# gardnerzhou/CHAP

Hardware: AMD Instinct MI355X
Metric: training volumes/sec (2D 256^2 bs24) (higher is better)
Workload: dtype bf16; 1 GPU; ACDC 2D DualDecoder bs=24 (12 lab + 12 unlab) 256x256, 1 perturb step(s), N_v=U; global_batch=24, parallelism=dp1, hip_graph=True, losses_finite=True

## Files before the change

chap_amd/csrc/conv_api.hip:

```cpp
#include <cstdlib>
#include <atomic>
#include "common.h"
#include "launch.h"

int chap_conv_launch_kpar_bf16(const chap_conv_params* p, int KC, int cpar, hipStream_t s);
int chap_conv_launch_wp_bf16(const chap_conv_params* p, int KC, hipStream_t s);
#define DECL_GEOM(dt, g) int chap_conv_launch_##dt##_g##g(const chap_conv_params* p, int KC, int NT, int MR, hipStream_t s);
DECL_GEOM(bf16, 1) DECL_GEOM(bf16, 2) DECL_GEOM(bf16, 3) DECL_GEOM(bf16, 4) DECL_GEOM(bf16, 5)
DECL_GEOM(f32, 1) DECL_GEOM(f32, 2) DECL_GEOM(f32, 3) DECL_GEOM(f32, 4) DECL_GEOM(f32, 5)
typedef int (*conv_launch_fn)(const chap_conv_params*, int, int, int, hipStream_t);

struct conv_blocking { int KC, GPT, NP, STEPS, nchunks, ntiles; };

static conv_blocking blocking_for(int Ck, int taps, int Cout_logical, int dtype) {
    conv_blocking b;
    b.KC = (Ck >= 32 && Ck % 32 == 0) ? 32 : 16;
    (void)dtype;
    {
        static int kc16_maxc = -1, kc16_maxc2 = -1;
        if (kc16_maxc < 0) { const char* e = getenv("CHAP_CONV_KC16_MAXC"); kc16_maxc = (e && atoi(e) > 0) ? atoi(e) : 1 << 20; }
        if (kc16_maxc2 < 0) { const char* e = getenv("CHAP_CONV_KC16_MAXC2D"); kc16_maxc2 = (e && atoi(e) > 0) ? atoi(e) : 0; }
        if (taps == 27 && Ck >= 32 && Ck <= kc16_maxc) b.KC = 16;
        if (taps == 9 && Ck >= 32 && Ck <= kc16_maxc2) b.KC = 16;
    }
// ... 54 lines not shown
                   "chap_conv_fwd: input dims (%d,%d,%d) do not match grid (%d,%d,%d) stride %d", p->ID, p->IH, p->IW, p->D, p->H, p->W, p->stride);
    if (p->dims == 3 && (p->src[0].keep || (p->nsrc > 1 && p->src[1].keep))) { chap_set_error("chap_conv_fwd: element keep masks are built for 2D only (3D: channel multipliers)"); return CHAP_EUNSUPPORTED; }
    if (p->out_mode == 1) CHAP_CHECK_ARG(p->out_Cn > 0 && p->out_Cn % 16 == 0 && p->Cout % p->out_Cn == 0, "chap_conv_fwd: depth-to-space needs Cn%%16==0");
    if (!p->out_planar) CHAP_CHECK_ARG(p->out_ld % 4 == 0 && p->out_coff % 4 == 0, "chap_conv_fwd: out_ld/out_coff must be multiples of 4");
    if (p->out2) CHAP_CHECK_ARG(p->out_mode == 0 && !p->out_planar && !p->out_f32 && (p->Cout & 3) == 0 && p->out2_from > 0 && p->out2_from % 16 == 0 && p->out2_from < p->Cout &&
                                p->ksize == 3 && p->stride == 1, "chap_conv_fwd: out2 needs a channel-last k3 s1 output, out2_from %% 16 == 0 inside (0, Cout)");
    const int Ck = p->combine == 0 ? p->src[0].C + (p->nsrc > 1 ? p->src[1].C : 0) : p->src[0].C;
    const int taps = p->ksize * p->ksize * (p->dims == 3 ? p->ksize : 1);
    conv_blocking b = blocking_for(Ck, taps, p->Cout, p->dtype);
    CHAP_CHECK_ARG(Ck % b.KC == 0, "chap_conv_fwd: K channels %d not a multiple of %d", Ck, b.KC);
    const bool d3 = p->dims == 3;
    int geom;
    if (p->ksize == 3 && p->stride == 1) geom = d3 ? 2 : 1;
    else if (p->ksize == 1 && p->stride == 1) geom = 3;
    else if (p->ksize == 2 && p->stride == 2) geom = d3 ? 5 : 4;
    else { chap_set_error("chap_conv_fwd: unsupported (ksize=%d, stride=%d)", p->ksize, p->stride); return CHAP_EUNSUPPORTED; }
    if (p->combine == 1 && p->nsrc == 2 && geom != 2 && geom != 1) { chap_set_error("chap_conv_fwd: add-combine is built for k3 s1 only"); return CHAP_EUNSUPPORTED; }
    int NT = b.ntiles >= 4 ? 4 : (b.ntiles >= 2 ? 2 : 1);
    int MR = (geom == 2 || geom == 5) ? 1 : 2;
    const bool bf = p->dtype == CHAP_BF16;
    if (geom == 2 && bf) {
        const long bricks = (long)p->N * cdiv(p->D, 4) * cdiv(p->H, 4) * cdiv(p->W, 16);
        if (bricks >= 64) {
            MR = 4;
            if (NT > 2) NT = 2;
            while (NT > 1 && bricks * cdiv(b.ntiles, NT) < 128) NT >>= 1;
        } else if (b.KC == 32 && NT > 2) {
            NT = 2;
        }
    }
    if (geom == 1 || geom == 3) {
        auto blocks = [&](int mr, int nt) { return (long)p->N * p->D * cdiv(p->H, 4 * mr) * cdiv(p->W, 16) * cdiv(b.ntiles, nt); };
        if (geom == 1 && bf && b.KC == 32 && b.ntiles >= 4) {
            MR = 2; NT = 2;
        } else if (geom == 1 && b.KC == 16 && blocks(4, NT) >= 512) MR = 4;
        else if (blocks(2, NT) >= 384) MR = 2;
        else {
            MR = 1;
            while (NT > 1 && blocks(1, NT) < 384) NT >>= 1;
        }
    }
    {
        const char* ent = getenv("CHAP_CONV_NT"); const char* emr = getenv("CHAP_CONV_MR"); const char* emc = getenv("CHAP_CONV_MINC");
        const int minc = emc ? atoi(emc) : 64;
        if ((geom == 1 || geom == 2) && Ck >= minc) {
            if (ent && atoi(ent) > 0 && atoi(ent) <= b.ntiles) NT = atoi(ent);
            if (emr && atoi(emr) > 0) MR = atoi(emr);
        }
    }
    if (p->dtype == CHAP_BF16 && geom == 3 && p->out_planar && p->Cout <= 8 && p->nsrc == 1 && Ck == 16 && p->src[0].C == 16 && !p->stats && p->out_mode == 0) {
        const long total = (long)p->N * p->D * p->H * p->W;
        return chap_launch<chap_conv_params, conv_head1x1_kernel<bf16_t>, 256>(dim3(chap_blocks(total, 4096)), dim3(256), 0, (hipStream_t)stream, *p, "chap_conv_fwd(head)");
    }
    if (p->dtype == CHAP_BF16 && geom == 1 && p->out_mode == 0 && !p->out_planar && !p->out_f32 && (p->Cout & 15) == 0 && p->Cout <= 64 && p->combine == 0 &&
        Ck == b.KC && (p->nsrc == 1 || (b.KC == 32 && p->src[0].C == 16 && p->src[1].C == 16))) {
        const char* ew = getenv("CHAP_CONV_WP");
        const long wp_min = ew ? atol(ew) : 1;
        const long t4 = (long)p->N * cdiv(p->H, 4) * cdiv(p->W, 16);
        if (wp_min > 0 && t4 >= wp_min) return chap_conv_launch_wp_bf16(p, b.KC, (hipStream_t)stream);
    }
    if (p->dtype == CHAP_BF16 && (geom == 1 || geom == 2) && p->out_mode == 0 && !p->out_planar && (p->Cout & 3) == 0 && !p->out2 &&
        (p->nsrc == 1 || (p->combine == 0 && p->src[0].C % b.KC == 0)) && !(d3 && (p->src[0].keep || (p->nsrc > 1 && p->src[1].keep)))) {
        const char* ek = getenv("CHAP_CONV_KPAR");
        const int mode = ek ? atoi(ek) : 2;
        const int cpar = b.nchunks % 4 == 0 ? 4 : (b.nchunks % 2 == 0 ? 2 : 0);
        const long kblocks = (long)p->N * p->D * cdiv(p->H, d3 ? 4 : 8) * cdiv(p->W, 16) * cdiv(b.ntiles, 2);
        const char* ekm = getenv("CHAP_CONV_KPAR_MAX");
        const long kmax = ekm ? atol(ekm) : 800;
        if (cpar && Ck >= 64 && (mode == 1 || (mode == 2 && d3 && kblocks <= kmax))) return chap_conv_launch_kpar_bf16(p, b.KC, cpar, (hipStream_t)stream);
    }
    static const conv_launch_fn table[2][5] = {
        {chap_conv_launch_f32_g1, chap_conv_launch_f32_g2, chap_conv_launch_f32_g3, chap_conv_launch_f32_g4, chap_conv_launch_f32_g5},
        {chap_conv_launch_bf16_g1, chap_conv_launch_bf16_g2, chap_conv_launch_bf16_g3, chap_conv_launch_bf16_g4, chap_conv_launch_bf16_g5}};
    if (p->dtype != CHAP_BF16 && p->dtype != CHAP_F32) { chap_set_error("chap_conv_fwd: dtype=%d", p->dtype); return CHAP_EINVAL; }
    return table[p->dtype == CHAP_BF16][geom - 1](p, b.KC, NT, MR, (hipStream_t)stream);
}

struct pack_geom { int Ck, Ck_real, Cn_logical, ctaps; };
static int pack_geometry(const chap_pack_params* p, pack_geom* g) {
    switch (p->kind) {
        case CHAP_PACK_CONV_FWD:     g->Ck = p->Cin;  g->Cn_logical = p->Cout;           g->ctaps = p->taps; break;
        case CHAP_PACK_CONV_DGRAD:   g->Ck = p->Cout; g->Cn_logical = p->Cin;            g->ctaps = p->taps; break;
        case CHAP_PACK_DECONV_FWD:   g->Ck = p->Cin;  g->Cn_logical = p->taps * p->Cout; g->ctaps = 1;       break;
        case CHAP_PACK_DECONV_DGRAD: g->Ck = p->Cout; g->Cn_logical = p->Cin;            g->ctaps = p->taps; break;
        case CHAP_PACK_DOWN_DGRAD:   g->Ck = p->Cout; g->Cn_logical = p->taps * p->Cin;  g->ctaps = 1;       break;
        default: chap_set_error("chap_pack: kind=%d", p->kind); return CHAP_EINVAL;
    }
    g->Ck_real = g->Ck;
    g->Ck = (g->Ck + 15) / 16 * 16;
    return CHAP_OK;
}

template <typename T>
__device__ __forceinline__ void pack_body(const float* __restrict__ w, T* __restrict__ out, int kind, int Cin, int Cout, int taps,
                                          int KC, int GPT, int NP, int STEPS, int nchunks, int ntiles, int Cn_logical, int Ck_real,
                                          long first, long stride) {
    const long total = (long)nchunks * STEPS * ntiles * 64;
    const int PPS = STEPS * 4;
    for (long q = first; q < total; q += stride) {
        const int pp = (int)(q % PPS);
        long r = q / PPS;
        const int n16 = (int)(r & 15); r >>= 4;
        const int nt = (int)(r % ntiles);
        const int chunk = (int)(r / ntiles);
        const int step = pp >> 2, g = pp & 3;
        const long i = ((long)(chunk * STEPS + step) * ntiles + nt) * 64 + g * 16 + n16;
        const int nl = nt * 16 + n16;
        float v[8];
// ... 90 lines not shown
```

chap_amd/csrc/conv_wp.h:

```cpp
#pragma once
#include "conv_kernel.h"
#include "wgrad_wp.h"

constexpr int CWP_AFFC = 64;

template <int KC, int NT>
__host__ __device__ constexpr size_t conv_wp_lds_bytes() {
    typedef conv_geom<3, 1, false, 1, false> G;
    constexpr int GPT = KC / 8, NP = G::NTAPS * GPT, STEPS = (NP + 3) / 4;
    return (size_t)STEPS * NT * 512 * sizeof(bf16_t)
           + 4 * ((size_t)G::HP * pix_stride<bf16_t, KC>() + HALO_DUMMY) * sizeof(bf16_t)
           + 4 * 2 * 16 * NT * sizeof(float) + 2 * CWP_AFFC * sizeof(float) + 2 * 16 * NT * sizeof(float);
}

template <int KC, int NT, bool LANESEL>
__device__ __forceinline__ void conv_wp_kernel(const chap_conv_params& P) {
    typedef bf16_t T;
    typedef conv_geom<3, 1, false, 1, false> G;
    typedef typename frag<T>::type F;
    constexpr int GPT = KC / 8, PS = pix_stride<T, KC>();
    constexpr int NP = G::NTAPS * GPT, STEPS = (NP + 3) / 4;
    constexpr int UNITS = (G::HP * GPT + 63) / 64;
    constexpr int ROWS = G::TH;
    constexpr size_t HB = (size_t)G::HP * PS + HALO_DUMMY;
    static_assert((HB * sizeof(T)) % 16 == 0, "the float4 reads of bc need a 16-byte aligned tail");
    extern __shared__ __attribute__((aligned(16))) char smem[];
    T* wlds = (T*)smem;
    const int lane = threadIdx.x & 63, wave = threadIdx.x >> 6;
    T* halo = wlds + (size_t)STEPS * NT * 512 + wave * HB;
    float* bstat = (float*)(wlds + (size_t)STEPS * NT * 512 + 4 * HB);
    float* aff = bstat + 4 * 2 * 16 * NT;
    float* bc = aff + 2 * CWP_AFFC;
    const int px = lane & 15, g = lane >> 4;
    const int tiles_x = (P.W + G::TW - 1) / G::TW, tiles_y = (P.H + G::TH - 1) / G::TH;
    const long ntiles = (long)P.N * tiles_y * tiles_x;
    const int ntiles_total = (P.Cout + 15) >> 4;
    const int nt0 = blockIdx.y * NT;
    const bool one = P.nsrc == 1;
    const bool plain = P.src[0].scale == nullptr && !P.src[0].act && P.src[0].keep == nullptr && P.src[0].chan_mul == nullptr &&
                       (one || (P.src[1].scale == nullptr && !P.src[1].act && P.src[1].keep == nullptr && P.src[1].chan_mul == nullptr));
    const src_scalars s0 = make_scalars(P.src[0]);
    const src_scalars s1 = make_scalars(one ? P.src[0] : P.src[1]);
    const bool do_stats = P.stats != nullptr;

    const int nb = gridDim.x;
    const int NG = nb < 8 ? nb : 8;
    const int xcd = blockIdx.x % NG;
    const int sj = ((int)blockIdx.x / NG) * 4 + wave;
    const int bpx = ((nb + NG - 1 - xcd) / NG) * 4;
    const long per = (ntiles + NG - 1) / NG;
    const long t_lo = per * xcd, t_hi = t_lo + per < ntiles ? t_lo + per : ntiles;
    const long my_tiles = (bpx > 0 && t_lo + sj < t_hi) ? (t_hi - t_lo - sj + bpx - 1) / bpx : 0;
    const long last_tile = t_lo + sj + (my_tiles > 0 ? my_tiles - 1 : 0) * bpx;
    auto tile_of = [&](long k) __attribute__((always_inline)) { const long t = t_lo + sj + k * bpx; return t < last_tile ? t : last_tile; };

    unit_desc<UNITS> U;
    make_units_wave<G, GPT, PS, UNITS>(U, P.IH, P.IW, lane);
    halo_regs<T, UNITS, false, true> R;
    int n = 0, y0 = 0, x0 = 0, nn = 0, ny0 = 0, nx0 = 0;
    auto issue = [&](long tile) __attribute__((always_inline)) {
        int z0_;
        tile_coords<G::TH, G::TW, 1>(tile, tiles_x, tiles_y, 1, nn, z0_, ny0, nx0);
        halo_issue_impl<T, G, false, 1, KC, false, UNITS, LANESEL, false>(R, U, s0, s1, 1, P.IH, P.IW, nn, 0, ny0, nx0, 0);
    };
    if (my_tiles > 0) issue(tile_of(0));
    float asc[2], ash[2];
    {
        const int s_ = threadIdx.x >> 5, c = threadIdx.x & 31;
        const chap_src_t& S = P.src[(s_ < P.nsrc && s_ < 2) ? s_ : 0];
        const int cc = c < S.C ? c : 0;
        asc[0] = S.scale ? S.scale[cc] : 1.f; ash[0] = S.scale ? S.shift[cc] : 0.f;
        asc[1] = 0.f; ash[1] = 0.f;
    }
    const long wstep = (long)ntiles_total * 64 * 8;
    constexpr int WPT = (STEPS * NT * 64 + 255) / 256;
    F wreg[WPT];
#pragma unroll
    for (int k = 0; k < WPT; ++k) {
        const unsigned i = min((unsigned)(threadIdx.x + 256 * k), (unsigned)(STEPS * NT * 64 - 1));
        const unsigned ln = i & 63u, r = i >> 6, t = r % (unsigned)NT, step = r / (unsigned)NT;
        const unsigned tt = nt0 + (int)t < ntiles_total ? t : 0u;
        wreg[k] = frag<T>::load((const T*)P.wpacked + (long)step * wstep + ((long)(nt0 + tt) * 64 + ln) * 8);
    }
    float ssum[NT][4], ssq[NT][4];
#pragma unroll
    for (int t = 0; t < NT; ++t)
#pragma unroll
        for (int j = 0; j < 4; ++j) { ssum[t][j] = 0.f; ssq[t][j] = 0.f; }
    float bcv = 0.f;
    if (threadIdx.x < 2 * 16 * NT) {
        const int which = threadIdx.x / (16 * NT), nl = nt0 * 16 + (int)threadIdx.x % (16 * NT);
        const float* srcp = which == 0 ? P.bias : (do_stats ? P.stats_shift : nullptr);
        if (srcp != nullptr && nl < P.Cout) bcv = srcp[nl];
    }
    if (threadIdx.x < 64) {
        const int s_ = threadIdx.x >> 5, c = threadIdx.x & 31;
        aff[s_ * CWP_AFFC + c] = asc[0]; aff[s_ * CWP_AFFC + CWP_AFFC / 2 + c] = ash[0];
    }
    if (threadIdx.x < 2 * 16 * NT) bc[threadIdx.x] = bcv;
#pragma unroll
    for (int k = 0; k < WPT; ++k) {
        const unsigned i = threadIdx.x + 256 * k;
        if (i < (unsigned)(STEPS * NT * 64)) {
            const unsigned t = (i >> 6) % (unsigned)NT;
            frag<T>::store(wlds + (size_t)i * 8, (nt0 + (int)t < ntiles_total) ? wreg[k] : frag<T>::zero());
        }
    }
    int xoff[STEPS];
#pragma unroll
    for (int step = 0; step < STEPS; ++step) {
        const int p = step * 4 + g;
        const int tap = p / GPT, cgl = p % GPT;
        const int dx = tap % 3, dy = tap / 3;
        xoff[step] = p < NP ? ((dy * G::HW) + px + dx) * PS + cgl * 8 : -1;
    }
    int ooff[NT];
#pragma unroll
    for (int t = 0; t < NT; ++t) {
        const int nl = (nt0 + t) * 16 + 4 * g;
        ooff[t] = px * P.out_ld + P.out_coff + ((P.out2 && nl >= P.out2_from) ? nl - P.out2_from : nl);
    }
    const int orow = P.W * P.out_ld;
    __syncthreads();
    if (my_tiles > 0) {
        halo_commit_impl<T, KC, false, UNITS, LANESEL, true, false, CWP_AFFC>(R, U, halo, s0, s1, aff, plain, nn, 0);
        for (long k = 0;; ++k) {
            n = nn; y0 = ny0; x0 = nx0;
            issue(tile_of(k + 1));
            f32x4 acc[ROWS][NT];
#pragma unroll
            for (int m = 0; m < ROWS; ++m)
#pragma unroll
                for (int t = 0; t < NT; ++t) acc[m][t] = (f32x4){0.f, 0.f, 0.f, 0.f};
#pragma unroll
            for (int step = 0; step < STEPS; ++step) {
                F wf[NT], xf[ROWS];
#pragma unroll
                for (int t = 0; t < NT; ++t) wf[t] = frag<T>::load(wlds + ((size_t)(step * NT + t) * 64 + lane) * 8);
                const int xo = xoff[step];
#pragma unroll
                for (int m = 0; m < ROWS; ++m) {
                    if (step * 4 + 3 < NP) xf[m] = frag<T>::load(halo + xo + m * (G::HW * PS));
                    else xf[m] = xo >= 0 ? frag<T>::load(halo + xo + m * (G::HW * PS)) : frag<T>::zero();
                }
#pragma unroll
                for (int m = 0; m < ROWS; ++m)
#pragma unroll
                    for (int t = 0; t < NT; ++t) mma8(acc[m][t], wf[t], xf[m]);
            }
            {
                const bool xok = x0 + px < P.W;
                const long o0 = (((long)n * P.H + y0) * P.W + x0) * P.out_ld;
                char* ob = (char*)P.out + o0 * (long)sizeof(T);
                char* ob2 = P.out2 ? (char*)P.out2 + o0 * (long)sizeof(T) : ob;
#pragma unroll
                for (int t = 0; t < NT; ++t) {
                    const bool cok = (nt0 + t) * 16 + 4 * g < P.Cout;
                    char* obt = (P.out2 && (nt0 + t) * 16 >= P.out2_from) ? ob2 : ob;
                    const float4 b4 = *(const float4*)(bc + t * 16 + 4 * g), c4 = *(const float4*)(bc + 16 * NT + t * 16 + 4 * g);
                    const float bj[4] = {b4.x, b4.y, b4.z, b4.w}, cj[4] = {c4.x, c4.y, c4.z, c4.w};
#pragma unroll
                    for (int m = 0; m < ROWS; ++m) {
                        const bool valid = xok && cok && (y0 + m < P.H);
                        float v[4];
#pragma unroll
                        for (int j = 0; j < 4; ++j) v[j] = acc[m][t][j] + bj[j];
                        if (do_stats) {
#pragma unroll
                            for (int j = 0; j < 4; ++j) { const float d = valid ? v[j] - cj[j] : 0.f; ssum[t][j] += d; ssq[t][j] += d * d; }
                        }
                        if (valid) st4((T*)(obt + (unsigned)(m * orow + ooff[t]) * (unsigned)sizeof(T)), v);
                    }
                }
            }
            if (k + 1 >= my_tiles) break;
            halo_commit_impl<T, KC, false, UNITS, LANESEL, true, false, CWP_AFFC>(R, U, halo, s0, s1, aff, plain, nn, 0);
        }
    }
    if (do_stats) {
#pragma unroll
        for (int t = 0; t < NT; ++t) {
#pragma unroll
            for (int j = 0; j < 4; ++j) {
                const float s = row16_sum(ssum[t][j]), q = row16_sum(ssq[t][j]);
                if (px == 0) {
                    bstat[(wave * 2 + 0) * 16 * NT + t * 16 + 4 * g + j] = s;
                    bstat[(wave * 2 + 1) * 16 * NT + t * 16 + 4 * g + j] = q;
                }
            }
        }
        __syncthreads();
        if (blockIdx.x == 0 && blockIdx.y == 0 && threadIdx.x == 0) *(int*)P.stats = (int)gridDim.x;
        float* st = P.stats + CHAP_STATS_HDR + (long)blockIdx.x * 2 * P.Cout;
        for (int i = threadIdx.x; i < 2 * 16 * NT; i += 256) {
            const int which = i / (16 * NT), kk = i % (16 * NT);
            const int nl = nt0 * 16 + kk;
            const float v = (bstat[(0 * 2 + which) * 16 * NT + kk] + bstat[(1 * 2 + which) * 16 * NT + kk]) + (bstat[(2 * 2 + which) * 16 * NT + kk] + bstat[(3 * 2 + which) * 16 * NT + kk]);
            if (nl < P.Cout) st[which * P.Cout + nl] = v;
        }
    }
}
```

chap_amd/csrc/conv_wp_bf16.hip:

```cpp
#include "conv_wp.h"
#include <atomic>
#include <cstdlib>

template <int KC, int NT, bool LANESEL>
static int conv_wp_launch(const chap_conv_params* p, hipStream_t stream) {
    typedef conv_geom<3, 1, false, 1, false> G;
    constexpr int MINW = KC == 16 ? (NT == 1 ? 4 : 3) : 2;
    const void* kern = chap_kernel<chap_conv_params, conv_wp_kernel<KC, NT, LANESEL>, 256, MINW>();
    const size_t lds = conv_wp_lds_bytes<KC, NT>();
    static std::atomic<int> attr_set[16];
    int dev = 0;
    if (hipGetDevice(&dev) != hipSuccess || dev < 0 || dev >= 16) dev = 0;
    if (!attr_set[dev].load(std::memory_order_acquire)) {
        if (lds > 48 * 1024) {
            hipError_t e = hipFuncSetAttribute(kern, hipFuncAttributeMaxDynamicSharedMemorySize, (int)lds);
            if (e != hipSuccess) { chap_set_error("conv(wp): hipFuncSetAttribute(%zu) failed: %s", lds, hipGetErrorString(e)); return CHAP_ELAUNCH; }
        }
        attr_set[dev].store(1, std::memory_order_release);
    }
    const long ntiles = (long)p->N * cdiv(p->H, G::TH) * cdiv(p->W, G::TW);
    const int gy = cdiv((p->Cout + 15) / 16, NT);
    const char* e = getenv("CHAP_CONV_WP_BPC");
    const long bpc = (e && atol(e) > 0) ? atol(e) : (KC == 16 ? 4 : 2);
    long gx = 256 * bpc / gy;
    const long need = (ntiles + 7) / 8;
    if (gx > need) gx = need;
    if (gx > CHAP_STATS_MAX_SLOTS) gx = CHAP_STATS_MAX_SLOTS;
    gx = gx >= 8 ? gx / 8 * 8 : (gx < 1 ? 1 : gx);
    return chap_launch_ptr<chap_conv_params>(kern, dim3((unsigned)gx, gy), dim3(256), lds, stream, *p, "chap_conv_fwd(wp)");
}

int chap_conv_launch_wp_bf16(const chap_conv_params* p, int KC, hipStream_t s) {
    const int nt = (p->Cout + 15) / 16;
    const bool two = p->nsrc == 2;
    if (KC == 16) {
        if (two) { chap_set_error("chap_conv_fwd(wp): two sources need a 32-channel chunk"); return CHAP_EUNSUPPORTED; }
        return nt == 1 ? conv_wp_launch<16, 1, false>(p, s) : conv_wp_launch<16, 2, false>(p, s);
    }
    if (nt == 1) return two ? conv_wp_launch<32, 1, true>(p, s) : conv_wp_launch<32, 1, false>(p, s);
    return two ? conv_wp_launch<32, 2, true>(p, s) : conv_wp_launch<32, 2, false>(p, s);
}
```

chap_amd/csrc/wgrad_api.hip:

```cpp
#include <cstdlib>
#include <cstdio>
#include "common.h"
#include "launch.h"

int chap_wgrad_launch_bf16(const chap_wgrad_params* p, int KC, int brick, float* ws, float* ws_db, int nsplit, int Ca, int Cb, hipStream_t s);
int chap_wgrad_launch_f32(const chap_wgrad_params* p, int KC, int brick, float* ws, float* ws_db, int nsplit, int Ca, int Cb, hipStream_t s);

struct wg_plan { int Ca, Cb, KC, taps, nsplit, brick; long ntiles; size_t slab, bytes; };

static int wg_make_plan(const chap_wgrad_params* p, wg_plan* q) {
    CHAP_CHECK_ARG(p->na == 1 || p->na == 2, "chap_wgrad: na=%d", p->na);
    q->Ca = p->combine == 0 ? p->a[0].C + (p->na > 1 ? p->a[1].C : 0) : p->a[0].C;
    q->Cb = p->b.C;
    CHAP_CHECK_ARG(q->Ca % 16 == 0 && q->Cb % 8 == 0, "chap_wgrad: Ca=%d must be a multiple of 16, Cb=%d of 8", q->Ca, q->Cb);
    q->KC = (q->Ca >= 32 && q->Ca % 32 == 0) ? 32 : 16;
    if (p->dtype == CHAP_F32 && p->ksize == 2) q->KC = 16;
    q->brick = 0;
    {
        const char* eb = getenv("CHAP_WGRAD_BRICK");
        const long min_bricks = eb ? atol(eb) : 16;
        const long bricks = (long)p->N * cdiv(p->D, 4) * cdiv(p->H, 4) * cdiv(p->W, 16);
        if (p->dims == 3 && p->ksize == 3 && p->stride == 1 && p->dtype == CHAP_BF16 && min_bricks > 0 && bricks >= min_bricks &&
            p->a[0].C <= 256 && (p->na < 2 || p->a[1].C <= 256) && p->b.C <= 256) { q->brick = 1; q->KC = 16; }
    }
    {
        const char* e = getenv("CHAP_WGRAD_WP");
        const long wp_min = e ? atol(e) : 1;
        const long t8 = (long)p->N * cdiv(p->H, 8) * cdiv(p->W, 16);
        if (p->dims == 2 && p->ksize == 3 && p->stride == 1 && p->combine == 0 && p->dtype == CHAP_BF16 && wp_min > 0 && t8 >= wp_min &&
            p->a[0].C <= 256 && p->a[0].C % 16 == 0 && (p->na < 2 || (p->a[1].C <= 256 && p->a[1].C % 16 == 0)) && p->b.C <= 256) { q->brick = 2; q->KC = 16; }
    }
    CHAP_CHECK_ARG(q->Ca % q->KC == 0, "chap_wgrad: Ca=%d not a multiple of %d", q->Ca, q->KC);
    q->taps = p->ksize * p->ksize * (p->dims == 3 ? p->ksize : 1);
    const bool small_tile = (p->dims == 3 && p->ksize >= 2);
    const int TH = small_tile ? 4 : 8;
    q->ntiles = (long)p->N * (q->brick == 1 ? cdiv(p->D, 4) : p->D) * cdiv(p->H, TH) * cdiv(p->W, 16);
    static int bn16_maxc = -1;
    if (bn16_maxc < 0) { const char* e = getenv("CHAP_WGRAD_BN16_MAXC"); bn16_maxc = (e && atoi(e) > 0) ? atoi(e) : 16; }
    const int bn = (q->Cb <= 16 || (q->brick == 1 && q->Cb <= bn16_maxc)) ? 16 : 32;
    const long pairs = (long)(q->Ca / q->KC) * cdiv(q->Cb, bn);
    long target = 256;
    const bool d3 = p->dims == 3;
    const char* env = getenv("CHAP_WGRAD_BLOCKS");
    if (env && atol(env) > 0) target = atol(env);
    else if (q->brick == 2) { static long wpb = -1; if (wpb < 0) { const char* e = getenv("CHAP_WGRAD_WP_BLOCKS"); wpb = (e && atol(e) > 0) ? atol(e) : 512; } target = wpb; }
    else if (p->ksize == 2) target = 256;
    else if (q->brick) { const char* eb2 = getenv("CHAP_WGRAD_BRICK_BLOCKS"); target = bn == 16 ? 512 : (eb2 && atol(eb2) > 0 ? atol(eb2) : 256); }
    else if (q->KC == 16) target = d3 ? 512 : 768;
    {
        const char* et = getenv("CHAP_WGRAD_TARGETS");
        long ta = 0, tb = 0, tc = 0;
        if (et && !(env && atol(env) > 0) && sscanf(et, "%ld,%ld,%ld", &ta, &tb, &tc) == 3 && p->ksize != 2 && !q->brick) {
            if (q->KC == 16) { if (!d3 && ta > 0) target = ta; }
            else if (!d3 && (p->na == 2 || q->Ca <= 32)) { if (tb > 0) target = tb; }
            else if (tc > 0) target = tc;
        }
    }
    long ns = target / pairs;
    if (ns < 1) ns = 1;
    if (ns > q->ntiles) ns = q->ntiles;
    q->slab = (size_t)q->taps * q->Ca * q->Cb * sizeof(float);
    const size_t cap = (size_t)96 << 20;
    while (ns > 1 && (size_t)ns * q->slab > cap) ns /= 2;
    q->nsplit = (int)ns;
    q->bytes = (size_t)q->nsplit * (q->slab + (size_t)q->Cb * sizeof(float));
    return CHAP_OK;
}

extern "C" size_t chap_wgrad_ws(const chap_wgrad_params* p) {
    wg_plan q;
    if (!p || wg_make_plan(p, &q)) return 0;
    return q.bytes;
}

struct wgrad_reduce_args { const float* ws; const float* ws_db; int nsplit, taps, Ca, Cb; float* dw; long s_tap, s_kc, s_kn; int kc_valid, kn_valid; float* db; int nb_dw; };
template <int E4>
__device__ __forceinline__ void wgrad_reduce_kernel(const wgrad_reduce_args& A) {
    const int bid = (int)blockIdx.x;
    const float* __restrict__ ws = A.ws; const float* __restrict__ ws_db = A.ws_db;
    const int nsplit = A.nsplit, taps = A.taps, Ca = A.Ca, Cb = A.Cb, kc_valid = A.kc_valid, kn_valid = A.kn_valid, nb_dw = A.nb_dw;
    float* dw = A.dw; float* db = A.db;
    const long s_tap = A.s_tap, s_kc = A.s_kc, s_kn = A.s_kn;
// ... 64 lines not shown
```

chap_amd/csrc/wgrad_wp.h:

```cpp
#pragma once
#include "wgrad_kernel.h"

constexpr int WP_AFFC = 512;

template <int KC, int MR, int BN>
__host__ __device__ constexpr size_t wgrad_wp_lds_bytes() {
    typedef conv_geom<3, 1, false, MR, false> G;
    return 4 * ((size_t)G::HP * pix_stride<bf16_t, KC>() + HALO_DUMMY + (size_t)G::TH * G::TW * wg_psb<bf16_t, BN>() + WG_BDUMMY) * sizeof(bf16_t)
           + 3 * WP_AFFC * sizeof(float) + 4 * BN * sizeof(float);
}

template <typename G, int GPT, int PS, int UNITS>
__device__ __forceinline__ void make_units_wave(unit_desc<UNITS>& U, int IH, int IW, int lane) {
    U.c8 = (lane % GPT) * 8;
#pragma unroll
    for (int j = 0; j < UNITS; ++j) {
        const int u = lane + 64 * j;
        U.hzyx[j] = UNIT_UNUSED; U.rel[j] = 0; U.lds[j] = G::HP * PS;
        if (u < G::HP * GPT) {
            const int pix = u / GPT, cgl = u % GPT;
            const int hx = pix % G::HW, hy = pix / G::HW;
            U.hzyx[j] = (hy << 10) | hx;
            U.rel[j] = hy * IW + hx;
            U.lds[j] = pix * PS + cgl * 8;
        }
    }
}

template <int KC, int MR, int BN>
__device__ __forceinline__ void wgrad_wp_kernel(const wgrad_args& A, int nb) {
    typedef bf16_t T;
    const chap_wgrad_params& P = A.P;
    float* __restrict__ ws = A.ws;
    float* __restrict__ ws_db = A.ws_db;
    const int nsplit = A.nsplit, Ca = A.Ca, Cb = A.Cb;
    typedef conv_geom<3, 1, false, MR, false> G;
    constexpr int TPX = G::TH * G::TW;
    typedef typename frag<T>::type F;
    constexpr int GPT = KC / 8, PS = pix_stride<T, KC>(), PSB = wg_psb<T, BN>();
    constexpr int KCT = KC / 16, NTB = BN / 16, CG = BN / 8;
    constexpr int PAIRS = G::NTAPS * KCT;
    constexpr int NKCH = TPX / 32;
    constexpr int UNITS = (G::HP * GPT + 63) / 64;
    constexpr int BUNITS = (TPX * CG + 63) / 64;
    constexpr size_t WBYTES = ((size_t)G::HP * PS + HALO_DUMMY + (size_t)TPX * PSB + WG_BDUMMY) * sizeof(T);
    constexpr int RP = (int)(WBYTES / (256 * sizeof(float))) < PAIRS ? (int)(WBYTES / (256 * sizeof(float))) : PAIRS;
    static_assert(RP >= 1, "tile region too small for the end-of-block reduction");
    extern __shared__ __attribute__((aligned(16))) char smem[];
    const int lane = threadIdx.x & 63, wave = threadIdx.x >> 6;
    T* halo = (T*)(smem + wave * WBYTES);
    T* bt = halo + (size_t)G::HP * PS + HALO_DUMMY;
    float* aff = (float*)(smem + 4 * WBYTES);
    float* dbred = aff + 3 * WP_AFFC;
    const int g = lane >> 4;
    const int split = blockIdx.x, chunk = blockIdx.y;
    const int tiles_x = (P.W + G::TW - 1) / G::TW, tiles_y = (P.H + G::TH - 1) / G::TH;
    const long ntiles = (long)P.N * tiles_y * tiles_x;
    const int NG = nsplit < 8 ? nsplit : 8;
    const int xcd = split % NG;
    const int sj = (split / NG) * 4 + wave;
    const int bpx = ((nsplit + NG - 1 - xcd) / NG) * 4;
    const long per = (ntiles + NG - 1) / NG;
    const long t_lo = per * xcd, t_hi = t_lo + per < ntiles ? t_lo + per : ntiles;
    const long my_tiles = (bpx > 0 && t_lo + sj < t_hi) ? (t_hi - t_lo - sj + bpx - 1) / bpx : 0;

    const src_scalars s0 = make_scalars(P.a[0]);
    const src_scalars s1 = make_scalars(P.na > 1 ? P.a[1] : P.a[0]);
    const src_scalars sb = make_scalars(P.b);
    const bool plainA = P.a[0].scale == nullptr && !P.a[0].act && P.a[0].keep == nullptr && P.a[0].chan_mul == nullptr &&
                        (P.na < 2 || (P.a[1].scale == nullptr && !P.a[1].act && P.a[1].keep == nullptr && P.a[1].chan_mul == nullptr));
    const bool plainB = P.b.scale == nullptr && !P.b.act && P.b.keep == nullptr && P.b.chan_mul == nullptr;

    unit_desc<UNITS> U;
    make_units_wave<G, GPT, PS, UNITS>(U, P.IH, P.IW, lane);
    int b_yx[BUNITS], b_rel[BUNITS], b_lds[BUNITS];
    const int bc8 = (lane & (CG - 1)) * 8;
    const int cbB = nb * BN + bc8;
    const bool bchan_ok = cbB < Cb;
    const int cbB_safe = bchan_ok ? cbB : 0;
#pragma unroll
    for (int j = 0; j < BUNITS; ++j) {
        const int u = lane + 64 * j;
        const int pix = u / CG;
        b_yx[j] = -1; b_rel[j] = 0; b_lds[j] = TPX * PSB;
        if (pix < TPX) {
            const int row = pix / G::TW, col = pix % G::TW;
            b_yx[j] = (row << 8) | col;
            b_rel[j] = row * P.W + col;
            b_lds[j] = pix * PSB + bc8;
        }
    }
    for (int s = 0; s < 3; ++s) {
        const chap_src_t& src = s == 2 ? P.b : P.a[s < P.na ? s : 0];
        const bool has = src.scale != nullptr;
        for (int c = threadIdx.x; c < src.C && c < WP_AFFC / 2; c += 256) {
            aff[s * WP_AFFC + c] = has ? src.scale[c] : 1.f;
            aff[s * WP_AFFC + WP_AFFC / 2 + c] = has ? src.shift[c] : 0.f;
        }
    }

    f32x4 acc[PAIRS][NTB];
#pragma unroll
    for (int i = 0; i < PAIRS; ++i)
#pragma unroll
        for (int t = 0; t < NTB; ++t) acc[i][t] = (f32x4){0.f, 0.f, 0.f, 0.f};
    float dbsum[8];
#pragma unroll
    for (int j = 0; j < 8; ++j) dbsum[j] = 0.f;
    const bool want_db = ws_db != nullptr && chunk == 0;

    struct pre_t { halo_regs<T, UNITS, false, true> R; F braw[BUNITS]; uint2 bkeep[BUNITS]; unsigned bok; int n; };
    pre_t S;
    f32x2 ba[4], bb2[4];

    auto issue = [&](pre_t& Q, long tile) __attribute__((always_inline)) {
        int n, z0, y0, x0;
        tile_coords<G::TH, G::TW, 1>(tile, tiles_x, tiles_y, 1, n, z0, y0, x0);
        Q.n = n;
        halo_issue_impl<T, G, false, 1, KC, false, UNITS, false, false>(Q.R, U, s0, s1, 1, P.IH, P.IW, n, 0, y0, x0, chunk);
        const long gp0 = ((long)n * P.H + y0) * P.W + x0;
        const char* bb = (const char*)sb.ptr + (gp0 * sb.ld + sb.coff + cbB_safe) * (long)sizeof(T);
        const unsigned ldb = sb.ld * sizeof(T);
        unsigned r[BUNITS];
        Q.bok = 0;
#pragma unroll
        for (int j = 0; j < BUNITS; ++j) {
            const int d = b_yx[j];
            const bool ok = d >= 0 && bchan_ok && y0 + (d >> 8) < P.H && x0 + (d & 255) < P.W;
            Q.bok |= ok ? (1u << j) : 0u;
            r[j] = ok ? (unsigned)b_rel[j] : 0u;
        }
#pragma unroll
        for (int j = 0; j < BUNITS; ++j) Q.braw[j] = frag<T>::load((const T*)(bb + __umul24(r[j], ldb)));
        if (sb.has_keep) {
            const uint8_t* kb = sb.keep + gp0 * sb.C + cbB_safe;
#pragma unroll
            for (int j = 0; j < BUNITS; ++j) Q.bkeep[j] = *(const uint2*)(kb + __umul24(r[j], (unsigned)sb.C));
        }
    };
    auto commit = [&](const pre_t& Q) __attribute__((always_inline)) {
        halo_commit_impl<T, KC, false, UNITS, false, true, false, WP_AFFC>(Q.R, U, halo, s0, s1, aff, plainA, Q.n, chunk);
        f32x2 a[4], b[4];
#pragma unroll
        for (int k = 0; k < 4; ++k) { a[k] = ba[k]; b[k] = bb2[k]; }
        if (sb.has_cm) {
            float bcm[8];
            ld8(sb.chan_mul + (long)Q.n * sb.C + cbB_safe, bcm);
#pragma unroll
            for (int k = 0; k < 4; ++k) { const f32x2 m = {bcm[2 * k], bcm[2 * k + 1]}; a[k] *= m; b[k] *= m; }
        }
#pragma unroll
        for (int j = 0; j < BUNITS; ++j) {
            T* dst = bt + b_lds[j];
            const bool ok = (Q.bok >> j) & 1u;
            if (plainB) {
                if (want_db) {
                    float v[8];
                    frag<T>::unpack(Q.braw[j], v);
#pragma unroll
                    for (int k = 0; k < 8; ++k) dbsum[k] += ok ? v[k] : 0.f;
                }
                frag<T>::store(dst, frag<T>::select(ok, Q.braw[j]));
                continue;
            }
            float v[8];
            frag<T>::unpack(Q.braw[j], v);
            affine_act8(v, a, b, sb.slope_eff);
            if (sb.has_keep) keep8(v, Q.bkeep[j], sb.keep_scale);
            if (want_db) {
#pragma unroll
                for (int k = 0; k < 8; ++k) dbsum[k] += ok ? v[k] : 0.f;
            }
            frag<T>::store(dst, frag<T>::select(ok, frag<T>::pack(v)));
        }
    };

    const int q = lane & 15, qq = q >> 2, pp = q & 3;
    const int rowl = g >> 1, xb = 8 * (g & 1);
    const int a_lane = (rowl * G::HW + xb + qq) * PS + 4 * pp;
    const int b_off = (rowl * G::TW + xb + qq) * PSB + 4 * pp;

    const long last_tile = t_lo + sj + (my_tiles > 0 ? my_tiles - 1 : 0) * bpx;
    auto tile_of = [&](long k) __attribute__((always_inline)) { const long t = t_lo + sj + k * bpx; return t < last_tile ? t : last_tile; };
    if (my_tiles > 0) issue(S, tile_of(0));
    __syncthreads();
#pragma unroll
    for (int k = 0; k < 4; ++k) {
        ba[k] = *(const f32x2*)(aff + 2 * WP_AFFC + cbB_safe + 2 * k);
        bb2[k] = *(const f32x2*)(aff + 2 * WP_AFFC + WP_AFFC / 2 + cbB_safe + 2 * k);
    }
    if (my_tiles > 0) commit(S);

    auto compute = [&]() __attribute__((always_inline)) {
        constexpr int NSTEP = NKCH * PAIRS, DEPTH = NSTEP < WG_DEPTH ? NSTEP : WG_DEPTH;
        auto load_a = [&](int st) __attribute__((always_inline)) -> uint4 {
            const int kc = st / PAIRS, i = st % PAIRS;
            const int tap = i / KCT, kct = i % KCT;
            const int dx = tap % 3, dy = tap / 3;
            const bf16_t* p = (const bf16_t*)halo + a_lane + (kc * 2 + dy) * (G::HW * PS) + dx * PS + kct * 16;
            const s16x4 lo = lds_tr16(p), hi = lds_tr16(p + 4 * PS);
            return __builtin_bit_cast(uint4, (s16x8){lo[0], lo[1], lo[2], lo[3], hi[0], hi[1], hi[2], hi[3]});
        };
        auto load_b = [&](int kc, uint4 (&bf)[NTB]) __attribute__((always_inline)) {
#pragma unroll
            for (int t = 0; t < NTB; ++t) {
                const bf16_t* bp = (const bf16_t*)bt + b_off + kc * (2 * G::TW * PSB) + t * 16;
                const s16x4 lo = lds_tr16(bp), hi = lds_tr16(bp + 4 * PSB);
                bf[t] = __builtin_bit_cast(uint4, (s16x8){lo[0], lo[1], lo[2], lo[3], hi[0], hi[1], hi[2], hi[3]});
            }
        };
        uint4 bf[2][NTB], af[DEPTH];
        load_b(0, bf[0]);
#pragma unroll
        for (int d = 0; d < DEPTH; ++d) af[d] = load_a(d);
#pragma unroll
        for (int st = 0; st < NSTEP; ++st) {
            const int kc = st / PAIRS, i = st % PAIRS;
            if (i == 0 && kc + 1 < NKCH) load_b(kc + 1, bf[(kc + 1) & 1]);
            const uint4 a = af[st % DEPTH];
#pragma unroll
            for (int t = 0; t < NTB; ++t) mma8(acc[i][t], a, bf[kc & 1][t]);
            if (st + DEPTH < NSTEP) af[st % DEPTH] = load_a(st + DEPTH);
        }
    };
    if (my_tiles > 0) {
        for (long k = 0;; ++k) {
            issue(S, tile_of(k + 1));
// ... 45 lines not shown
```

Measured before the change: 4003 volumes/s.

## Route planar fp32 head convs through wave-private kernel; pixel-owned halo staging in wgrad

Extends the wave-private 3x3 conv forward kernel with a PLANAR variant. The 16-channel, fp32, planar-output head convolutions can now use it instead of the generic geometry kernel, writing NCHW fp32 output with bias directly. The wgrad wave-private kernel switches halo staging to pixel-owned units (each lane loads all channel groups of one pixel) with explicit wavefront LDS fences, and the forward kernel gets the same option behind a compile flag that is off by default. This aims to cut generic-kernel overhead for the heads and simplify halo address math, at the cost of new code paths and a different synchronisation pattern.

```diff
diff --git a/chap_amd/csrc/conv_api.hip b/chap_amd/csrc/conv_api.hip
--- a/chap_amd/csrc/conv_api.hip
+++ b/chap_amd/csrc/conv_api.hip
@@ -130,8 +130,10 @@
         const long total = (long)p->N * p->D * p->H * p->W;
         return chap_launch<chap_conv_params, conv_head1x1_kernel<bf16_t>, 256>(dim3(chap_blocks(total, 4096)), dim3(256), 0, (hipStream_t)stream, *p, "chap_conv_fwd(head)");
     }
-    if (p->dtype == CHAP_BF16 && geom == 1 && p->out_mode == 0 && !p->out_planar && !p->out_f32 && (p->Cout & 15) == 0 && p->Cout <= 64 && p->combine == 0 &&
-        Ck == b.KC && (p->nsrc == 1 || (b.KC == 32 && p->src[0].C == 16 && p->src[1].C == 16))) {
+    const bool wp_cl = !p->out_planar && !p->out_f32 && (p->Cout & 15) == 0 && p->Cout <= 64 && (p->nsrc == 1 || (b.KC == 32 && p->src[0].C == 16 && p->src[1].C == 16));
+    const char* eh = getenv("CHAP_CONV_WP_HEAD");
+    const bool wp_head = !(eh && atoi(eh) == 0) && p->out_planar && p->out_f32 && p->Cout <= 16 && b.KC == 16 && p->nsrc == 1 && !p->stats && !p->out2 && (long)p->Cout * p->H * p->W < (1l << 31);
+    if (p->dtype == CHAP_BF16 && geom == 1 && p->D == 1 && p->out_mode == 0 && p->combine == 0 && Ck == b.KC && (wp_cl || wp_head)) {
         const char* ew = getenv("CHAP_CONV_WP");
         const long wp_min = ew ? atol(ew) : 1;
         const long t4 = (long)p->N * cdiv(p->H, 4) * cdiv(p->W, 16);
diff --git a/chap_amd/csrc/conv_wp.h b/chap_amd/csrc/conv_wp.h
--- a/chap_amd/csrc/conv_wp.h
+++ b/chap_amd/csrc/conv_wp.h
@@ -3,26 +3,33 @@
 #include "wgrad_wp.h"
 
 constexpr int CWP_AFFC = 64;
+#ifndef CHAP_CONV_WP_PXO
+#define CHAP_CONV_WP_PXO 0
+#endif
 
 template <int KC, int NT>
 __host__ __device__ constexpr size_t conv_wp_lds_bytes() {
     typedef conv_geom<3, 1, false, 1, false> G;
     constexpr int GPT = KC / 8, NP = G::NTAPS * GPT, STEPS = (NP + 3) / 4;
     return (size_t)STEPS * NT * 512 * sizeof(bf16_t)
-           + 4 * ((size_t)G::HP * pix_stride<bf16_t, KC>() + HALO_DUMMY) * sizeof(bf16_t)
+           + 4 * ((size_t)G::HP * pix_stride<bf16_t, KC>() + WP_HALO_DUMMY) * sizeof(bf16_t)
            + 4 * 2 * 16 * NT * sizeof(float) + 2 * CWP_AFFC * sizeof(float) + 2 * 16 * NT * sizeof(float);
 }
 
-template <int KC, int NT, bool LANESEL>
+template <int KC, int NT, bool LANESEL, bool PLANAR = false>
 __device__ __forceinline__ void conv_wp_kernel(const chap_conv_params& P) {
     typedef bf16_t T;
     typedef conv_geom<3, 1, false, 1, false> G;
     typedef typename frag<T>::type F;
     constexpr int GPT = KC / 8, PS = pix_stride<T, KC>();
     constexpr int NP = G::NTAPS * GPT, STEPS = (NP + 3) / 4;
-    constexpr int UNITS = (G::HP * GPT + 63) / 64;
+    constexpr bool PXO = CHAP_CONV_WP_PXO && KC == 16;
+    constexpr int PIX = (G::HP + 63) / 64;
+    constexpr int UNITS = PXO ? PIX * GPT : (G::HP * GPT + 63) / 64;
+    static_assert(!PXO || UNITS == (G::HP * GPT + 63) / 64, "pixel-owned staging takes no more registers than one unit per (lane, j)");
+    static_assert(!PLANAR || (KC == 16 && NT == 1 && !LANESEL), "the planar heads: one 16-channel chunk, one 16-wide output tile");
     constexpr int ROWS = G::TH;
-    constexpr size_t HB = (size_t)G::HP * PS + HALO_DUMMY;
+    constexpr size_t HB = (size_t)G::HP * PS + WP_HALO_DUMMY;
     static_assert((HB * sizeof(T)) % 16 == 0, "the float4 reads of bc need a 16-byte aligned tail");
     extern __shared__ __attribute__((aligned(16))) char smem[];
     T* wlds = (T*)smem;
@@ -41,7 +48,7 @@
                        (one || (P.src[1].scale == nullptr && !P.src[1].act && P.src[1].keep == nullptr && P.src[1].chan_mul == nullptr));
     const src_scalars s0 = make_scalars(P.src[0]);
     const src_scalars s1 = make_scalars(one ? P.src[0] : P.src[1]);
-    const bool do_stats = P.stats != nullptr;
+    const bool do_stats = !PLANAR && P.stats != nullptr;
 
     const int nb = gridDim.x;
     const int NG = nb < 8 ? nb : 8;
@@ -54,14 +61,22 @@
     const long last_tile = t_lo + sj + (my_tiles > 0 ? my_tiles - 1 : 0) * bpx;
     auto tile_of = [&](long k) __attribute__((always_inline)) { const long t = t_lo + sj + k * bpx; return t < last_tile ? t : last_tile; };
 
-    unit_desc<UNITS> U;
-    make_units_wave<G, GPT, PS, UNITS>(U, P.IH, P.IW, lane);
+    unit_desc<PXO ? PIX : UNITS> U;
+    if constexpr (PXO) make_pixels_wave<G, PS, PIX>(U, P.IW, lane);
+    else make_units_wave<G, GPT, PS, UNITS>(U, P.IH, P.IW, lane);
     halo_regs<T, UNITS, false, true> R;
     int n = 0, y0 = 0, x0 = 0, nn = 0, ny0 = 0, nx0 = 0;
     auto issue = [&](long tile) __attribute__((always_inline)) {
         int z0_;
         tile_coords<G::TH, G::TW, 1>(tile, tiles_x, tiles_y, 1, nn, z0_, ny0, nx0);
-        halo_issue_impl<T, G, false, 1, KC, false, UNITS, LANESEL, false>(R, U, s0, s1, 1, P.IH, P.IW, nn, 0, ny0, nx0, 0);
+        if constexpr (PXO) halo_issue_px<T, G, KC, PIX, true>(R, U, s0, s0, P.IH, P.IW, nn, ny0, nx0, 0);
+        else halo_issue_impl<T, G, false, 1, KC, false, UNITS, LANESEL, false>(R, U, s0, s1, 1, P.IH, P.IW, nn, 0, ny0, nx0, 0);
+    };
+    auto commit = [&]() __attribute__((always_inline)) {
+        wave_lds_acquire();
+        if constexpr (PXO) halo_commit_px<T, KC, PIX, true, CWP_AFFC>(R, U, halo, s0, s0, aff, plain, nn, 0);
+        else halo_commit_impl<T, KC, false, UNITS, LANESEL, true, false, CWP_AFFC>(R, U, halo, s0, s1, aff, plain, nn, 0);
+        wave_lds_release();
     };
     if (my_tiles > 0) issue(tile_of(0));
     float asc[2], ash[2];
@@ -123,7 +138,7 @@
     const int orow = P.W * P.out_ld;
     __syncthreads();
     if (my_tiles > 0) {
-        halo_commit_impl<T, KC, false, UNITS, LANESEL, true, false, CWP_AFFC>(R, U, halo, s0, s1, aff, plain, nn, 0);
+        commit();
         for (long k = 0;; ++k) {
             n = nn; y0 = ny0; x0 = nx0;
             issue(tile_of(k + 1));
@@ -148,6 +163,20 @@
 #pragma unroll
                     for (int t = 0; t < NT; ++t) mma8(acc[m][t], wf[t], xf[m]);
             }
+            if constexpr (PLANAR) {
+                const bool xok = x0 + px < P.W;
+                const unsigned plane = (unsigned)(P.H * P.W);
+                float* ob = (float*)P.out + ((long)n * P.Cout * P.H + y0) * P.W + x0;
+                const float4 b4 = *(const float4*)(bc + 4 * g);
+                const float bj[4] = {b4.x, b4.y, b4.z, b4.w};
+#pragma unroll
+                for (int m = 0; m < ROWS; ++m) {
+                    const bool valid = xok && (y0 + m < P.H);
+#pragma unroll
+                    for (int j = 0; j < 4; ++j)
+                        if (valid && 4 * g + j < P.Cout) ob[(unsigned)(4 * g + j) * plane + (unsigned)(m * P.W + px)] = acc[m][0][j] + bj[j];
+                }
+            } else
             {
                 const bool xok = x0 + px < P.W;
                 const long o0 = (((long)n * P.H + y0) * P.W + x0) * P.out_ld;
@@ -174,7 +203,7 @@
                 }
             }
             if (k + 1 >= my_tiles) break;
-            halo_commit_impl<T, KC, false, UNITS, LANESEL, true, false, CWP_AFFC>(R, U, halo, s0, s1, aff, plain, nn, 0);
+            commit();
         }
     }
     if (do_stats) {
diff --git a/chap_amd/csrc/conv_wp_bf16.hip b/chap_amd/csrc/conv_wp_bf16.hip
--- a/chap_amd/csrc/conv_wp_bf16.hip
+++ b/chap_amd/csrc/conv_wp_bf16.hip
@@ -2,11 +2,11 @@
 #include <atomic>
 #include <cstdlib>
 
-template <int KC, int NT, bool LANESEL>
+template <int KC, int NT, bool LANESEL, bool PLANAR = false>
 static int conv_wp_launch(const chap_conv_params* p, hipStream_t stream) {
     typedef conv_geom<3, 1, false, 1, false> G;
     constexpr int MINW = KC == 16 ? (NT == 1 ? 4 : 3) : 2;
-    const void* kern = chap_kernel<chap_conv_params, conv_wp_kernel<KC, NT, LANESEL>, 256, MINW>();
+    const void* kern = chap_kernel<chap_conv_params, conv_wp_kernel<KC, NT, LANESEL, PLANAR>, 256, MINW>();
     const size_t lds = conv_wp_lds_bytes<KC, NT>();
     static std::atomic<int> attr_set[16];
     int dev = 0;
@@ -33,6 +33,10 @@
 int chap_conv_launch_wp_bf16(const chap_conv_params* p, int KC, hipStream_t s) {
     const int nt = (p->Cout + 15) / 16;
     const bool two = p->nsrc == 2;
+    if (p->out_planar) {
+        if (KC != 16 || two || nt != 1 || !p->out_f32 || p->stats || p->out2) { chap_set_error("chap_conv_fwd(wp): planar output needs one 16-channel source, Cout <= 16, fp32, no statistics"); return CHAP_EUNSUPPORTED; }
+        return conv_wp_launch<16, 1, false, true>(p, s);
+    }
     if (KC == 16) {
         if (two) { chap_set_error("chap_conv_fwd(wp): two sources need a 32-channel chunk"); return CHAP_EUNSUPPORTED; }
         return nt == 1 ? conv_wp_launch<16, 1, false>(p, s) : conv_wp_launch<16, 2, false>(p, s);
diff --git a/chap_amd/csrc/wgrad_api.hip b/chap_amd/csrc/wgrad_api.hip
--- a/chap_amd/csrc/wgrad_api.hip
+++ b/chap_amd/csrc/wgrad_api.hip
@@ -27,7 +27,7 @@
         const char* e = getenv("CHAP_WGRAD_WP");
         const long wp_min = e ? atol(e) : 1;
         const long t8 = (long)p->N * cdiv(p->H, 8) * cdiv(p->W, 16);
-        if (p->dims == 2 && p->ksize == 3 && p->stride == 1 && p->combine == 0 && p->dtype == CHAP_BF16 && wp_min > 0 && t8 >= wp_min &&
+        if (p->dims == 2 && p->D == 1 && p->ksize == 3 && p->stride == 1 && p->combine == 0 && p->dtype == CHAP_BF16 && wp_min > 0 && t8 >= wp_min &&
             p->a[0].C <= 256 && p->a[0].C % 16 == 0 && (p->na < 2 || (p->a[1].C <= 256 && p->a[1].C % 16 == 0)) && p->b.C <= 256) { q->brick = 2; q->KC = 16; }
     }
     CHAP_CHECK_ARG(q->Ca % q->KC == 0, "chap_wgrad: Ca=%d not a multiple of %d", q->Ca, q->KC);
diff --git a/chap_amd/csrc/wgrad_wp.h b/chap_amd/csrc/wgrad_wp.h
--- a/chap_amd/csrc/wgrad_wp.h
+++ b/chap_amd/csrc/wgrad_wp.h
@@ -2,11 +2,12 @@
 #include "wgrad_kernel.h"
 
 constexpr int WP_AFFC = 512;
+constexpr int WP_HALO_DUMMY = 16;
 
 template <int KC, int MR, int BN>
 __host__ __device__ constexpr size_t wgrad_wp_lds_bytes() {
     typedef conv_geom<3, 1, false, MR, false> G;
-    return 4 * ((size_t)G::HP * pix_stride<bf16_t, KC>() + HALO_DUMMY + (size_t)G::TH * G::TW * wg_psb<bf16_t, BN>() + WG_BDUMMY) * sizeof(bf16_t)
+    return 4 * ((size_t)G::HP * pix_stride<bf16_t, KC>() + WP_HALO_DUMMY + (size_t)G::TH * G::TW * wg_psb<bf16_t, BN>() + WG_BDUMMY) * sizeof(bf16_t)
            + 3 * WP_AFFC * sizeof(float) + 4 * BN * sizeof(float);
 }
 
@@ -26,6 +27,118 @@
         }
     }
 }
+
+
+template <typename G, int PS, int PIX>
+__device__ __forceinline__ void make_pixels_wave(unit_desc<PIX>& U, int IW, int lane) {
+    U.c8 = 0;
+#pragma unroll
+    for (int j = 0; j < PIX; ++j) {
+        const int pix = lane + 64 * j;
+        U.hzyx[j] = UNIT_UNUSED; U.rel[j] = 0; U.lds[j] = G::HP * PS;
+        if (pix < G::HP) {
+            const int hx = pix % G::HW, hy = pix / G::HW;
+            U.hzyx[j] = (hy << 10) | hx;
+            U.rel[j] = hy * IW + hx;
+            U.lds[j] = pix * PS;
+        }
+    }
+}
+
+template <typename T, typename G, int KC, int PIX, bool ONE>
+__device__ __forceinline__ void halo_issue_px(halo_regs<T, PIX * (KC / 8), false, true>& R, const unit_desc<PIX>& U, const src_scalars& s0, const src_scalars& s1,
+                                              int IH, int IW, int n, int y0, int x0, int chunk) {
+    constexpr int GPT = KC / 8;
+    static_assert(8 * GPT <= WP_HALO_DUMMY, "the dummy slot behind the halo takes all units of an unused pixel");
+    const int gy0 = y0 - G::PAD, gx0 = x0 - G::PAD;
+    const long gp0 = ((long)n * IH + gy0) * IW + gx0;
+    const int loy = max(0, -gy0), hiy = min(G::HH, IH - gy0), lox = max(0, -gx0), hix = min(G::HW, IW - gx0);
+    const unsigned PA = (512u << 20) | ((unsigned)(512 - loy) << 10) | (unsigned)(512 - lox);
+    const unsigned PB = (511u << 20) | ((unsigned)(512 - hiy) << 10) | (unsigned)(512 - hix);
+    const unsigned rsafe = G::PAD * IW + G::PAD;
+    const int cb = chunk * KC;
+    const bool second = ONE ? false : cb >= s0.C;
+    const int cs = second ? cb - s0.C : cb;
+    const int ld = second ? s1.ld : s0.ld;
+    const long dptr = (const char*)s1.ptr - (const char*)s0.ptr;
+    const char* base = (const char*)s0.ptr + (second ? dptr : 0l) + (gp0 * ld + (second ? s1.coff : s0.coff) + cs) * (long)sizeof(T);
+    const unsigned ldb = ld * sizeof(T);
+    unsigned okm = 0, r[PIX];
+#pragma unroll
+    for (int j = 0; j < PIX; ++j) {
+        const unsigned d = (unsigned)U.hzyx[j];
+        const bool ok = (((d + PA) ^ (d + PB)) & UNIT_GUARD) == UNIT_GUARD;
+        okm |= ok ? (1u << j) : 0u;
+        r[j] = ok ? (unsigned)U.rel[j] : rsafe;
+    }
+    R.ok = okm;
+#pragma unroll
+    for (int j = 0; j < PIX; ++j) {
+        const T* px = (const T*)(base + __umul24(r[j], ldb));
+#pragma unroll
+        for (int h = 0; h < GPT; ++h) R.raw[j * GPT + h] = frag<T>::load(px + 8 * h);
+    }
+    const bool hk = second ? s1.has_keep : s0.has_keep;
+    if (!hk) {
+#pragma unroll
+        for (int j = 0; j < PIX * GPT; ++j) R.keep[j] = make_uint2(0u, 0u);
+    } else {
+        const int kC = second ? s1.C : s0.C;
+        const uint8_t* kb = (second ? s1.keep : s0.keep) + (gp0 * kC + cs);
+#pragma unroll
+        for (int j = 0; j < PIX; ++j) {
+            const uint8_t* kp = kb + __umul24(r[j], (unsigned)kC);
+#pragma unroll
+            for (int h = 0; h < GPT; ++h) R.keep[j * GPT + h] = *(const uint2*)(kp + 8 * h);
+        }
+    }
+}
+
+template <typename T, int KC, int PIX, bool ONE, int AFFC>
+__device__ __forceinline__ void halo_commit_px(const halo_regs<T, PIX * (KC / 8), false, true>& R, const unit_desc<PIX>& U, T* halo, const src_scalars& s0, const src_scalars& s1,
+                                               const float* aff, bool plain, int n, int chunk) {
+    constexpr int GPT = KC / 8;
+    if (plain) {
+#pragma unroll
+        for (int j = 0; j < PIX; ++j)
+#pragma unroll
+            for (int h = 0; h < GPT; ++h) frag<T>::store(halo + U.lds[j] + 8 * h, frag<T>::select((R.ok >> j) & 1u, R.raw[j * GPT + h]));
+        return;
+    }
+    const int cb = chunk * KC;
+    const bool second = ONE ? false : cb >= s0.C;
+    const float se = second ? s1.slope_eff : s0.slope_eff;
+    const bool hk = second ? s1.has_keep : s0.has_keep;
+    const float ks = second ? s1.keep_scale : s0.keep_scale;
+    const bool hcm = second ? s1.has_cm : s0.has_cm;
+#pragma unroll
+    for (int h = 0; h < GPT; ++h) {
+        aff_regs<false> A;
+        load_aff<KC, false, ONE, AFFC>(A, aff, 8 * h, s0.C, chunk, false);
+        f32x2 a[4], b[4];
+#pragma unroll
+        for (int k = 0; k < 4; ++k) { a[k] = A.a[k]; b[k] = A.b[k]; }
+        if (hcm) {
+            const int cs = second ? cb - s0.C : cb;
+            const float* cp = second ? s1.chan_mul + (long)n * s1.C + cs : s0.chan_mul + (long)n * s0.C + cs;
+            float cm[8];
+            ld8(cp + 8 * h, cm);
+#pragma unroll
+            for (int k = 0; k < 4; ++k) { const f32x2 m = {cm[2 * k], cm[2 * k + 1]}; a[k] *= m; b[k] *= m; }
+        }
+#pragma unroll
+        for (int j = 0; j < PIX; ++j) {
+            float v[8];
+            frag<T>::unpack(R.raw[j * GPT + h], v);
+            affine_act8(v, a, b, se);
+            if (hk) keep8(v, R.keep[j * GPT + h], ks);
+            frag<T>::store(halo + U.lds[j] + 8 * h, frag<T>::select((R.ok >> j) & 1u, frag<T>::pack(v)));
+        }
+    }
+}
+
+__device__ __forceinline__ void wave_lds_release() { __builtin_amdgcn_fence(__ATOMIC_RELEASE, "wavefront"); __builtin_amdgcn_wave_barrier(); }
+__device__ __forceinline__ void wave_lds_acquire() { __builtin_amdgcn_wave_barrier(); __builtin_amdgcn_fence(__ATOMIC_ACQUIRE, "wavefront"); }
 
 template <int KC, int MR, int BN>
 __device__ __forceinline__ void wgrad_wp_kernel(const wgrad_args& A, int nb) {
@@ -41,15 +154,16 @@
     constexpr int KCT = KC / 16, NTB = BN / 16, CG = BN / 8;
     constexpr int PAIRS = G::NTAPS * KCT;
     constexpr int NKCH = TPX / 32;
-    constexpr int UNITS = (G::HP * GPT + 63) / 64;
+    constexpr int PIX = (G::HP + 63) / 64, UNITS = PIX * GPT;
+    static_assert(UNITS == (G::HP * GPT + 63) / 64, "pixel-owned staging takes no more registers than one unit per (lane, j)");
     constexpr int BUNITS = (TPX * CG + 63) / 64;
-    constexpr size_t WBYTES = ((size_t)G::HP * PS + HALO_DUMMY + (size_t)TPX * PSB + WG_BDUMMY) * sizeof(T);
+    constexpr size_t WBYTES = ((size_t)G::HP * PS + WP_HALO_DUMMY + (size_t)TPX * PSB + WG_BDUMMY) * sizeof(T);
     constexpr int RP = (int)(WBYTES / (256 * sizeof(float))) < PAIRS ? (int)(WBYTES / (256 * sizeof(float))) : PAIRS;
     static_assert(RP >= 1, "tile region too small for the end-of-block reduction");
     extern __shared__ __attribute__((aligned(16))) char smem[];
     const int lane = threadIdx.x & 63, wave = threadIdx.x >> 6;
     T* halo = (T*)(smem + wave * WBYTES);
-    T* bt = halo + (size_t)G::HP * PS + HALO_DUMMY;
+    T* bt = halo + (size_t)G::HP * PS + WP_HALO_DUMMY;
     float* aff = (float*)(smem + 4 * WBYTES);
     float* dbred = aff + 3 * WP_AFFC;
     const int g = lane >> 4;
@@ -71,8 +185,8 @@
                         (P.na < 2 || (P.a[1].scale == nullptr && !P.a[1].act && P.a[1].keep == nullptr && P.a[1].chan_mul == nullptr));
     const bool plainB = P.b.scale == nullptr && !P.b.act && P.b.keep == nullptr && P.b.chan_mul == nullptr;
 
-    unit_desc<UNITS> U;
-    make_units_wave<G, GPT, PS, UNITS>(U, P.IH, P.IW, lane);
+    unit_desc<PIX> U;
+    make_pixels_wave<G, PS, PIX>(U, P.IW, lane);
     int b_yx[BUNITS], b_rel[BUNITS], b_lds[BUNITS];
     const int bc8 = (lane & (CG - 1)) * 8;
     const int cbB = nb * BN + bc8;
@@ -117,7 +231,7 @@
         int n, z0, y0, x0;
         tile_coords<G::TH, G::TW, 1>(tile, tiles_x, tiles_y, 1, n, z0, y0, x0);
         Q.n = n;
-        halo_issue_impl<T, G, false, 1, KC, false, UNITS, false, false>(Q.R, U, s0, s1, 1, P.IH, P.IW, n, 0, y0, x0, chunk);
+        halo_issue_px<T, G, KC, PIX, false>(Q.R, U, s0, s1, P.IH, P.IW, n, y0, x0, chunk);
         const long gp0 = ((long)n * P.H + y0) * P.W + x0;
         const char* bb = (const char*)sb.ptr + (gp0 * sb.ld + sb.coff + cbB_safe) * (long)sizeof(T);
         const unsigned ldb = sb.ld * sizeof(T);
@@ -139,7 +253,8 @@
         }
     };
     auto commit = [&](const pre_t& Q) __attribute__((always_inline)) {
-        halo_commit_impl<T, KC, false, UNITS, false, true, false, WP_AFFC>(Q.R, U, halo, s0, s1, aff, plainA, Q.n, chunk);
+        wave_lds_acquire();
+        halo_commit_px<T, KC, PIX, false, WP_AFFC>(Q.R, U, halo, s0, s1, aff, plainA, Q.n, chunk);
         f32x2 a[4], b[4];
 #pragma unroll
         for (int k = 0; k < 4; ++k) { a[k] = ba[k]; b[k] = bb2[k]; }
@@ -173,6 +288,7 @@
             }
             frag<T>::store(dst, frag<T>::select(ok, frag<T>::pack(v)));
         }
+        wave_lds_release();
     };
 
     const int q = lane & 15, qq = q >> 2, pp = q & 3;
```

After: 3971 volumes/s, median of 2. About the same (-0.8%).
